# gkm2708/gym-lmaze

Measured on AMD Instinct MI355X. Metric: env steps/sec (whole node), 1M parallel 11x11 mazes at 1/2/4/8 MI355X, higher is better.
Workload: dtype int32

## Files before the change

gym-lmaze_amd/csrc/lmaze_foveal.hip:

```cpp
#include <cstdio>
#include <cstring>
#include <type_traits>

#include "lmaze_foveal_defs.h"

namespace lmaze {

#ifdef LMAZE_FOVEAL_WAVES
#define LMAZE_FOVEAL_ATTR __attribute__((amdgpu_waves_per_eu(LMAZE_FOVEAL_WAVES)))
#else
#define LMAZE_FOVEAL_ATTR
#endif
template <int VARIANT, int MODE, int EPB, int GT, bool AR>
__global__ __launch_bounds__(LMAZE_BLOCK) LMAZE_FOVEAL_ATTR void foveal_kernel(const FovealArgs a) {
    constexpr bool ROLL = false, REC = false;
    const FovealRoll ro{};
#define LMAZE_FOVEAL_BODY_SITE
#include "lmaze_foveal_body.h"
#undef LMAZE_FOVEAL_BODY_SITE
}

template <int VARIANT, int EPB, int GT, bool AR>
__global__ __launch_bounds__(LMAZE_BLOCK) __attribute__((amdgpu_waves_per_eu(4))) void foveal_rollout_kernel(const FovealArgs a, const FovealRoll ro) {
    constexpr bool ROLL = true, REC = false;
    constexpr int MODE = FM_STEP;
#define LMAZE_FOVEAL_BODY_SITE
#include "lmaze_foveal_body.h"
#undef LMAZE_FOVEAL_BODY_SITE
}

template <int VARIANT, int EPB, int GT, bool AR>
__global__ __launch_bounds__(LMAZE_BLOCK)
__attribute__((amdgpu_waves_per_eu(VARIANT == LMAZE_VARIANT_V1 || VARIANT == LMAZE_VARIANT_V2 ? 6 : 4)))
void foveal_rollout_kernel(const FovealArgs a, const FovealRollObs ro) {
    constexpr bool ROLL = true, REC = true;
    constexpr int MODE = FM_STEP;
#define LMAZE_FOVEAL_BODY_SITE
#include "lmaze_foveal_body.h"
#undef LMAZE_FOVEAL_BODY_SITE
}

__global__ __launch_bounds__(LMAZE_BLOCK) void safe_goal_kernel(const FovealArgs a, int32_t* out_goal) {
    const int64_t e = (int64_t)blockIdx.x * LMAZE_BLOCK + threadIdx.x;
    if (e >= a.n) return;
    const int G = a.p.grid;
    const uint8_t* lay = a.layouts + (size_t)clampi(a.b.layout_id[e], 0, a.p.n_layouts - 1) * G * G;
    const int bx = a.b.ball_xy[2 * e], by = a.b.ball_xy[2 * e + 1];
    const uint4 d = env_draw(a.seed, a.epoch, a.env_base + e);
    unsigned ok = 0;
    for (int c = 0; c < W25; ++c) {
        const int x = bx - 2 + c / FOV, y = by - 2 + c % FOV;
        const bool in = x >= 0 && y >= 0 && x < G && y < G;
        if (in && lay[x * G + y] != 'W') ok |= 1u << c;
    }
    int pick = 12;
    const int cnt = __popc(ok);
    if (cnt > 0) {
        int k = (int)__umulhi(d.x, (uint32_t)cnt);
        for (int c = 0; c < W25; ++c)
            if (ok & (1u << c)) {
                if (k == 0) { pick = c; break; }
                --k;
            }
    }
    out_goal[e] = pick;
}

struct ExpandPlanesArgs {
    const float* planes;
    float* out;
    int64_t n;
    int32_t channels, g, expansion;
};

__global__ __launch_bounds__(LMAZE_BLOCK) void expand_planes_kernel(const ExpandPlanesArgs a) {
    extern __shared__ int4 lds4[];
    const int g = a.g, E = a.expansion, C = a.channels;
    const int PC = g * g, S = g * E, PLANE = S * S, L = C * PLANE;
    float* src = reinterpret_cast<float*>(lds4);
    uint16_t* rowmap = reinterpret_cast<uint16_t*>(src + C * PC);
    uint16_t* colmap = rowmap + S;
    const int tid = threadIdx.x;
    for (int64_t i = blockIdx.x; i < a.n; i += gridDim.x) {
        __syncthreads();
        for (int k = tid; k < C * PC; k += LMAZE_BLOCK) src[k] = a.planes[(size_t)i * C * PC + k];
        for (int k = tid; k < S; k += LMAZE_BLOCK) {
            rowmap[k] = (uint16_t)((k / E) * g);
            colmap[k] = (uint16_t)(k / E);
        }
        __syncthreads();
        const size_t B = (size_t)i * L;
        const size_t a0 = (B + 3) & ~(size_t)3, a1 = (B + L) & ~(size_t)3;
        auto value = [&](int local) -> float {
            const int c = local / PLANE;
            const int rem = local - c * PLANE;
            const int row = rem / S, col = rem - row * S;
            return src[c * PC + rowmap[row] + colmap[col]];
        };
        if (tid < (int)(a0 - B)) a.out[B + tid] = value(tid);
        if (tid < (int)(B + L - a1)) a.out[a1 + tid] = value((int)(a1 - B) + tid);
        const int nq = (int)((a1 - a0) >> 2);
        float4* out4 = reinterpret_cast<float4*>(a.out + a0);
        const int head = (int)(a0 - B);
        for (int q = tid; q < nq; q += LMAZE_BLOCK) {
            const int local = head + (q << 2);
            int c = local / PLANE;
            int rem = local - c * PLANE;
            int row = rem / S, col = rem - row * S;
            float v[4];
#pragma unroll
            for (int j = 0; j < 4; ++j) {
                v[j] = src[c * PC + rowmap[row] + colmap[col]];
                if (++col == S) {
                    col = 0;
                    if (++row == S) { row = 0; ++c; }
                }
            }
            out4[q] = make_float4(v[0], v[1], v[2], v[3]);
        }
    }
}

template <int GT, int ET, bool NT>
__global__ __launch_bounds__(LMAZE_BLOCK) void expand_planes_stream_kernel(const ExpandPlanesArgs a, int chunk_floats) {
    constexpr int PC = GT * GT, S = GT * ET, PLANE = S * S;
    extern __shared__ int4 lds4[];
    float* src = reinterpret_cast<float*>(lds4);
    const int tid = threadIdx.x;
    const int64_t total = a.n * (int64_t)a.channels * PLANE;
    const int64_t f0 = (int64_t)blockIdx.x * chunk_floats;
    const int len = (int)min((int64_t)chunk_floats, total - f0);
    const int64_t p0 = f0 / PLANE;
    const int off0 = (int)(f0 - p0 * PLANE);
    const int np = (off0 + len + PLANE - 1) / PLANE;
    for (int k = tid; k < np * PC; k += LMAZE_BLOCK) src[k] = a.planes[(size_t)p0 * PC + k];
    __syncthreads();
    float* dst = a.out + f0;
    static_assert(ET >= 4, "four consecutive output columns span at most two cells");
    for (int q = tid; (q << 2) < len; q += LMAZE_BLOCK) {
        const int local = off0 + (q << 2);
        const int p = local / PLANE;
        const int rem = local - p * PLANE;
        const int row = rem / S, col = rem - row * S;
        const float* r0 = src + p * PC + (row / ET) * GT;
        const int k0 = col / ET;
        const float v0 = r0[k0], v1 = r0[k0 + 1];
        int row1 = row + 1, p1 = p;
        if (row1 == S) { row1 = 0; ++p1; }
        const float vw = src[p1 * PC + (row1 / ET) * GT];
        const int edge = (k0 + 1) * ET;
        float v[4];
#pragma unroll
        for (int j = 0; j < 4; ++j) {
            const int cj = col + j;
            v[j] = cj >= S ? vw : (cj >= edge ? v1 : v0);
        }
        const int count = len - (q << 2);
        if (count >= 4) {
            if (NT) {
                typedef float f4 __attribute__((ext_vector_type(4)));
                f4 t = {v[0], v[1], v[2], v[3]};
                stream_store16(reinterpret_cast<f4*>(dst) + q, t);
            } else {
                reinterpret_cast<float4*>(dst)[q] = make_float4(v[0], v[1], v[2], v[3]);
// ... 517 lines not shown
```

gym-lmaze_amd/csrc/lmaze_foveal_body.h:

```cpp
#ifndef LMAZE_FOVEAL_BODY_SITE
#error "lmaze_foveal_body.h is the body of the foveal kernels: it is included only inside them, in lmaze_foveal.hip and lmaze_foveal_policy.hip"
#endif
#ifdef LMAZE_FOVEAL_POLICY_SITE
#define LMAZE_POL 1
#else
#define LMAZE_POL 0
#endif
    constexpr bool V1 = VARIANT == LMAZE_VARIANT_V1, V5 = VARIANT == LMAZE_VARIANT_V5;
    constexpr bool V4 = VARIANT == LMAZE_VARIANT_V4 || V5;
    constexpr int C = V1 ? 4 : (V4 ? 7 : 5);
    constexpr int PLACE_U = V5 ? 1 : 4;
    constexpr int PERENV = C * W25;
    const int G = GT ? GT : a.p.grid, CELLS = G * G, L = V1 ? 1 : a.p.n_layouts;

    extern __shared__ int4 lds4[];
    uint32_t* obits = reinterpret_cast<uint32_t*>(lds4);
    uint32_t* lbits = obits + EPB * 8;
    int16_t* cen = reinterpret_cast<int16_t*>(lbits + EPB * 4);
    int32_t* flags = reinterpret_cast<int32_t*>(cen + EPB * 4);
    int16_t* rcen = reinterpret_cast<int16_t*>(flags + EPB);
    float* vwin = reinterpret_cast<float*>(rcen + EPB * 2);
    int32_t* clk = reinterpret_cast<int32_t*>(vwin + (V4 ? EPB * 2 * W25 : 0));
    int32_t* dlist = clk + (V4 ? EPB : 0);
    uint64_t* rowfree = reinterpret_cast<uint64_t*>(dlist + (V4 ? EPB : 0));
    uint64_t* rowgoal = rowfree + L * G;
    uint64_t* rowball = rowgoal + L * G;
    uint64_t* rowwall = rowball + L * G;
    uint64_t* rowx = rowwall + G;
    uint8_t* lays = reinterpret_cast<uint8_t*>(rowx + G);
#if LMAZE_POL
    uint8_t* ptab = lays + ((L * CELLS + 15) & ~15);
    const FovealPol pol = ro.pol;
    const bool pstage = pol.in_lds != 0;
#endif
    static_assert(PERENV <= 8 * 32 - 32 && 4 * W25 <= 4 * 32 - 4, "bit strings fit the 32 B / 16 B per env reserved for them");
    __shared__ int any_skip, ndense;

    const int tid = threadIdx.x;
    const int64_t nchunks = (a.n + EPB - 1) / EPB;
    int64_t chunk = blockIdx.x;
    int64_t blockbase = chunk * EPB;
    int nb = (int)min((int64_t)EPB, a.n - blockbase);
    if (tid == 0) { any_skip = 0; ndense = 0; }
    for (int i = tid; i < EPB * 12; i += LMAZE_BLOCK) obits[i] = 0u;
    if (V4) for (int i = tid; i < EPB * 2 * W25; i += LMAZE_BLOCK) vwin[i] = 0.0f;
    const uint64_t epoch = launch_epoch(a.epoch, a.epoch_in);
    if (MODE == FM_STEP && AR) pass_epoch_on(a.epoch_in, a.epoch_out);
    int warmed = 0;
    if (MODE == FM_STEP && !ROLL && a.nt) {
        warmed = warm_lines(a.action, a.n * 4, 256);
        if (!V5 || LMAZE_WARM_V4(a)) {
            warmed += warm_lines(a.b.ball_xy, a.n * 8, 256) + warm_lines(a.b.step_count, a.n * 4, 256);
            if (V1) warmed += warm_lines(a.b.fgoal_xy, a.n * 8, 256) + warm_lines(a.b.foveal_step_count, a.n * 4, 256);
            else warmed += warm_lines(a.b.goal_xy, a.n * 8, 256) + warm_lines(a.b.layout_id, a.n * 4, 256);
            if (V4) warmed += warm_lines(a.b.visit_clock, a.n * 4, 256);
            if (V5) warmed += warm_lines(a.b.fgoal_xy, a.n * 8, 256) + warm_lines(a.b.foveal_step_count, a.n * 4, 256) +
                              warm_lines(a.b.fovea_xy, a.n * 16, 256) + warm_lines(a.b.ball1_xy, a.n * 8, 256) +
                              warm_lines(a.b.last_xy, a.n * 8, 256) + warm_lines(a.b.foveal_goal, a.n * 4, 256) +
                              warm_lines(a.goal2, a.n * 4, 256);
        }
    }
    if (LMAZE_XP(a, 1)) {
    } else if (GT != 0) {
        constexpr int GG = GT ? GT : 1, RPW = 64 / GG, UNR = 8;
        const int wave = tid >> 6, lane = tid & 63, rows = L * G;
        const int rsub = lane / GG, y = lane - rsub * GG;
        const bool dwords = ((reinterpret_cast<uintptr_t>(a.layouts) | (uintptr_t)(L * CELLS)) & 3) == 0;
        uint32_t cw[2] = {0u, 0u};
        if (dwords) {
#pragma unroll
            for (int j = 0; j < 2; ++j)
                if (tid + j * LMAZE_BLOCK < (L * CELLS) >> 2) cw[j] = reinterpret_cast<const uint32_t*>(a.layouts)[tid + j * LMAZE_BLOCK];
        }
#if LMAZE_POL
        const bool pdwords = pstage && ((reinterpret_cast<uintptr_t>(pol.table) | (uintptr_t)(L * CELLS)) & 3) == 0;
        uint32_t pw[2] = {0u, 0u};
        if (pdwords) {
#pragma unroll
            for (int j = 0; j < 2; ++j)
                if (tid + j * LMAZE_BLOCK < (L * CELLS) >> 2) pw[j] = reinterpret_cast<const uint32_t*>(pol.table)[tid + j * LMAZE_BLOCK];
        }
#endif
        for (int r00 = 0; r00 < rows; r00 += UNR * 4 * RPW) {
            uint8_t cc[UNR];
#pragma unroll
            for (int u = 0; u < UNR; ++u) {
                const int row = r00 + (u * 4 + wave) * RPW + rsub;
                cc[u] = (rsub < RPW && row < rows) ? a.layouts[(size_t)row * G + y] : (uint8_t)0;
            }
#pragma unroll
            for (int u = 0; u < UNR; ++u) {
                const int row = r00 + (u * 4 + wave) * RPW + rsub;
                const bool in = rsub < RPW && row < rows;
                const uint8_t c = cc[u];
                const unsigned long long bf = __ballot(in && (c == 'B' || c == 'S' || c == 'X'));
                const unsigned long long bw = __ballot(in && c == 'W');
                const unsigned long long bx = __ballot(in && c == 'X');
                const unsigned long long bs = __ballot(in && c == 'S');
                if (in && y == 0) {
                    const int sh = rsub * GG;
                    const uint64_t keep = GG == 64 ? ~0ull : ((1ull << GG) - 1ull);
                    const uint64_t fr = (bf >> sh) & keep, wl = (bw >> sh) & keep, xx = (bx >> sh) & keep, ss = (bs >> sh) & keep;
                    rowfree[row] = fr;
                    if (V1) { rowwall[row] = wl; rowx[row] = xx; }
                    if (!V1 && (MODE == FM_RESET || (MODE == FM_STEP && AR))) {
                        const int x = row % G;
                        const uint64_t interior = (x >= 1 && x <= G - 2) ? (((1ull << (G - 2)) - 1ull) << 1) : 0ull;
                        rowgoal[row] = fr & ~ss & interior;
                        rowball[row] = fr & ~xx & interior;
                    }
                }
            }
        }
        if (dwords) {
#pragma unroll
            for (int j = 0; j < 2; ++j)
                if (tid + j * LMAZE_BLOCK < (L * CELLS) >> 2) reinterpret_cast<uint32_t*>(lays)[tid + j * LMAZE_BLOCK] = cw[j];
            for (int i = tid + 2 * LMAZE_BLOCK; i < (L * CELLS) >> 2; i += LMAZE_BLOCK)
                reinterpret_cast<uint32_t*>(lays)[i] = reinterpret_cast<const uint32_t*>(a.layouts)[i];
        } else {
            for (int i = tid; i < L * CELLS; i += LMAZE_BLOCK) lays[i] = a.layouts[i];
        }
#if LMAZE_POL
        if (pdwords) {
#pragma unroll
            for (int j = 0; j < 2; ++j)
                if (tid + j * LMAZE_BLOCK < (L * CELLS) >> 2) reinterpret_cast<uint32_t*>(ptab)[tid + j * LMAZE_BLOCK] = pw[j];
            for (int i = tid + 2 * LMAZE_BLOCK; i < (L * CELLS) >> 2; i += LMAZE_BLOCK)
                reinterpret_cast<uint32_t*>(ptab)[i] = reinterpret_cast<const uint32_t*>(pol.table)[i];
        } else if (pstage) {
            for (int i = tid; i < L * CELLS; i += LMAZE_BLOCK) ptab[i] = pol.table[i];
        }
#endif
    } else {
    for (int i = tid; i < L * CELLS; i += LMAZE_BLOCK) lays[i] = a.layouts[i];
#if LMAZE_POL
    if (pstage) for (int i = tid; i < L * CELLS; i += LMAZE_BLOCK) ptab[i] = pol.table[i];
#endif
    __syncthreads();
    for (int i = tid; i < L * G; i += LMAZE_BLOCK) {
        uint64_t fr = 0, wl = 0, xx = 0;
        for (int y = 0; y < G; ++y) {
            const uint8_t c = lays[i * G + y];
            fr |= (uint64_t)(c == 'B' || c == 'S' || c == 'X') << y;
            wl |= (uint64_t)(c == 'W') << y;
            xx |= (uint64_t)(c == 'X') << y;
        }
        rowfree[i] = fr;
        if (V1) { rowwall[i] = wl; rowx[i] = xx; }
        if (!V1 && (MODE == FM_RESET || (MODE == FM_STEP && AR))) {
            uint64_t ss = 0;
            for (int y = 0; y < G; ++y) ss |= (uint64_t)(lays[i * G + y] == 'S') << y;
            const int x = i % G;
            const uint64_t interior = (x >= 1 && x <= G - 2) ? (((1ull << (G - 2)) - 1ull) << 1) : 0ull;
            rowgoal[i] = fr & ~ss & interior;
            rowball[i] = fr & ~xx & interior;
        }
    }
    }
    __syncthreads();

    int t = 0;
#define ROLL_ROW(e) (ROLL ? (int64_t)t * a.n + (e) : (e))
#define ROLL_EP (ROLL ? epoch + (uint64_t)t : epoch)
  for (;;) {
    for (int le = tid; le < (LMAZE_XP(a, 8) ? 0 : nb); le += LMAZE_BLOCK) {
        const int64_t e = blockbase + le;
        EnvRec r;
        r.skip = 0; r.flat = -1; r.action = -1; r.lid = 0; r.gx = r.gy = -9;
        r.b0x = r.b0y = r.b1x = r.b1y = r.f1x = r.f1y = 0; r.upd = 0; r.pad = 0;
        bool fresh = false, nostep = false;
        bool last_is_cur = true;
        int rx = 0, ry = 0;
        float row_r = -0.0f, row_fr = -0.0f;
        int row_d = 0, row_fd = 0;
        int bx = a.b.ball_xy[2 * e], by = a.b.ball_xy[2 * e + 1];
#if LMAZE_POL
        const int act_in = 0;
#else
        const int act_in = (MODE == FM_STEP) ? a.action[ROLL_ROW(e)] : 0;
#endif
        const int sc_ld = (MODE == FM_STEP) ? a.b.step_count[e] : 0;
        const int done_in = (MODE == FM_STEP && AR) ? a.b.done[e] : 0;
        const int goal2_in = (MODE == FM_STEP && AR && V5) ? a.goal2[ROLL_ROW(e)] : 0;
        const int vword = (V4 && !(V5 && MODE == FM_PLANNER)) ? a.b.visit_clock[e] : 0;
        const int vclock = vword & 0xff;
#if LMAZE_POL
        uint4 pr = make_uint4(0u, 0u, 0u, 0u);
        if (pol.epsilon != 0u) pr = policy_draw(a.seed, ROLL_EP, a.env_base + e);
#endif
        r.px = (int16_t)bx; r.py = (int16_t)by;
        if (MODE != FM_STEP && a.mask && !a.mask[e]) r.skip = 1;
        if (V1) {
            int fgx = a.b.fgoal_xy[2 * e], fgy = a.b.fgoal_xy[2 * e + 1];
            r.action = 1;
            if (MODE == FM_STEP) {
                int sc_in = sc_ld;
                if (AR && done_in) {
                    for (int c = 0; c < CELLS; ++c)
                        if (lays[c] == 'S') { bx = c / G; by = c % G; break; }
                    sc_in = 0;
                }
#if LMAZE_POL
                const int act = foveal_pol_action(pol, pstage, ptab, 0, bx, by, G, 1, 4, pr, ROLL_ROW(e));
#else
                const int act = act_in;
#endif
                const int sc = sc_in + 1;
                const int fsc = a.b.foveal_step_count[e] + 1;
                float fr = -0.0f, rw = -0.0f;
                bool local_done = false;
                int ox, oy;
                decode_action(act, ox, oy);
                const int tx = clampi(bx + ox, 0, G - 1), ty = clampi(by + oy, 0, G - 1);
                const uint8_t c = lays[tx * G + ty];
                if (c == 'W') {
                    rw = a.p.reward_wall; fr = a.p.reward_wall;
                } else if (c == 'B') {
                    bx = tx; by = ty;
                    rw = a.p.reward_move; fr = a.p.reward_move;
                    if (bx < fgx - 1 || bx > fgx + 2 || by < fgy - 1 || by > fgy + 2) {
                        local_done = true; fr = a.p.reward_wall;
                    } else if (by == fgy && bx == fgx) {
                        local_done = true; fr = a.p.reward_goal;
                    }
                } else if (c == 'X') {
                    bx = tx; by = ty;
                    rw = a.p.reward_goal;
                    if (by == fgy && bx == fgx) { local_done = true; fr = a.p.reward_goal; }
                    else fr = a.p.reward_move;
                }
                const bool done = (rw == a.p.reward_goal) || (sc == a.p.step_limit);
                const bool fdone = local_done || fr == a.p.reward_goal || fsc == a.p.foveal_step_limit || done;
                a.b.ball_xy[2 * e] = bx; a.b.ball_xy[2 * e + 1] = by;
                a.b.step_count[e] = sc; a.b.foveal_step_count[e] = fsc;
                a.b.reward[e] = rw; a.b.foveal_reward[e] = fr;
                a.b.done[e] = done ? 1 : 0; a.b.foveal_done[e] = fdone ? 1 : 0;
                row_r = rw; row_fr = fr; row_d = done; row_fd = fdone;
            } else if (MODE == FM_RESET && !r.skip) {
                if (a.place) {
                    for (int c = 0; c < CELLS; ++c)
                        if (lays[c] == 'S') { bx = c / G; by = c % G; break; }
                    a.b.ball_xy[2 * e] = bx; a.b.ball_xy[2 * e + 1] = by;
                }
                a.b.reward[e] = -0.0f; a.b.foveal_reward[e] = -0.0f;
                a.b.step_count[e] = 0;
                a.b.done[e] = 0; a.b.foveal_done[e] = 0;
                r.action = 0;
            } else if (MODE == FM_SETGOAL && !r.skip) {
                fgx = bx + a.action[2 * e] - 2;
                fgy = by + a.action[2 * e + 1] - 2;
                a.b.fgoal_xy[2 * e] = fgx; a.b.fgoal_xy[2 * e + 1] = fgy;
                a.b.foveal_step_count[e] = 0;
            }
            int flat = fgx * G + fgy;
            if (flat < 0) flat += CELLS;
            r.flat = (flat >= 0 && flat < CELLS) ? flat : -1;
        } else if (V5) {
            int lid = clampi(a.b.layout_id[e], 0, L - 1);
            int gx = a.b.goal_xy[2 * e], gy = a.b.goal_xy[2 * e + 1];
            int fg = a.b.foveal_goal[e];
            int f0x = a.b.fovea_xy[4 * e], f0y = a.b.fovea_xy[4 * e + 1];
            int f1x = a.b.fovea_xy[4 * e + 2], f1y = a.b.fovea_xy[4 * e + 3];
            int b1x = a.b.ball1_xy[2 * e], b1y = a.b.ball1_xy[2 * e + 1];
            int lx = a.b.last_xy[2 * e], ly = a.b.last_xy[2 * e + 1];
            if (MODE == FM_STEP) {
                const int act = act_in;
                int fgx = a.b.fgoal_xy[2 * e], fgy = a.b.fgoal_xy[2 * e + 1];
                int fsc = a.b.foveal_step_count[e];
                int sc_in = sc_ld;
                bool ld = a.b.foveal_done[e] != 0, gd = a.b.done[e] != 0;
                if (AR) {
                    const bool plan = ld || gd;
                    bool planned = false;
                    if (gd) {
                        const uint4 d = env_draw(a.seed, ROLL_EP, a.env_base + e);
                        lid = (int)__umulhi(d.z, (uint32_t)L);
                        int goal_cell, ball_cell;
                        place_goal_ball<PLACE_U>(rowgoal + lid * G, rowball + lid * G, G, d, goal_cell, ball_cell);
                        if (goal_cell >= 0) { gx = goal_cell / G; gy = goal_cell % G; }
                        if (ball_cell >= 0) { bx = ball_cell / G; by = ball_cell % G; }
                        a.b.layout_id[e] = lid;
                        a.b.goal_xy[2 * e] = gx; a.b.goal_xy[2 * e + 1] = gy;
                        fsc = 0; sc_in = 0; gd = false; ld = false;
                        fg = 12;
                        f0x = f1x = b1x = lx = fgx = bx; f0y = f1y = b1y = ly = fgy = by;
                        fresh = true;
                    }
                    if (plan) {
                        const int g = goal2_in;
                        if (g >= 0 && g < W25) {
                            fg = g;
                            sc_in = 0;
                            ld = false;
                            fgx = bx + g / FOV - 2; fgy = by + g % FOV - 2;
                            if (fsc > 0) { f1x = f0x; f1y = f0y; }
                            fsc += 1;
                            planned = true;
                        }
                    }
                    if (fresh || planned) {
                        a.b.foveal_goal[e] = fg;
                        a.b.fgoal_xy[2 * e] = fgx; a.b.fgoal_xy[2 * e + 1] = fgy;
                        a.b.fovea_xy[4 * e + 2] = f1x; a.b.fovea_xy[4 * e + 3] = f1y;
                        a.b.foveal_step_count[e] = fsc;
                    }
                }
                const uint8_t* lay = lays + lid * CELLS;
                b1x = bx; b1y = by;
                float lr = -0.0f, gr;
                const int sc = sc_in + 1;
                const int dx = (act == 0) - (act == 1), dy = (act == 2) - (act == 3);
                const int nx = bx + dx, ny = by + dy;
                const bool nin = nx >= 0 && ny >= 0 && nx < G && ny < G;
                const uint8_t c = nin ? lay[nx * G + ny] : (uint8_t)'W';
                if (c == 'W') {
                    lr = a.p.reward_wall;
// ... 131 lines not shown
                        if (fx >= G - 2) bx = G - 3;
                        if (fx <= 1) bx = 2;
                        if (fy >= G - 2) by = G - 3;
                        if (fy <= 1) by = 2;
                    }
                    const bool fin = fx >= 0 && fy >= 0 && fx < G && fy < G;
                    const uint8_t c = fin ? lay[fx * G + fy] : (uint8_t)'W';
                    if (fx == gx && fy == gy) rw = a.p.reward_goal;
                    else if (c == 'W') rw = a.p.reward_wall;
                    else if (c == 'B' || c == 'S') rw = a.p.reward_move;
                    a.b.ball_xy[2 * e] = bx; a.b.ball_xy[2 * e + 1] = by;
                    a.b.step_count[e] = sc;
                    a.b.reward[e] = rw;
                    a.b.done[e] = (rw == a.p.reward_goal || sc > a.p.step_limit) ? 1 : 0;
                    r.action = (int16_t)act;
                    row_r = rw; row_d = rw == a.p.reward_goal || sc > a.p.step_limit;
                }
            }
            r.lid = (int16_t)clampi(lid, 0, L - 1);
            r.gx = (int16_t)gx; r.gy = (int16_t)gy;
        }
        r.cx = (int16_t)bx; r.cy = (int16_t)by;
        uint32_t m[8];
        if (V1) {
            m[0] = 1u << 12;
            m[1] = window_bits(rowwall, G, r.cx, r.cy);
            m[2] = r.action ? (r.flat >= 0 ? onehot_bits(r.flat / G, r.flat % G, r.cx, r.cy) : 0u)
                            : window_bits(rowx, G, r.cx, r.cy);
            m[3] = window_bits(rowfree, G, r.cx, r.cy);
        } else {
            constexpr int PER = VARIANT == LMAZE_VARIANT_V2 ? 2 : 3;
            const uint64_t* rows = rowfree + r.lid * G;
            m[0] = window_bits(rows, G, r.cx, r.cy);
            m[1] = onehot_bits(r.gx, r.gy, r.cx, r.cy);
            m[PER] = (r.action >= 0 && r.action < W25) ? (1u << r.action) : 0u;
            m[PER + 1] = window_bits(rows, G, r.px, r.py);
            m[PER + 2] = onehot_bits(r.gx, r.gy, r.px, r.py);
            if (V5) {
                uint32_t lm[4];
                lm[0] = m[0];
                const int i0 = wrap5(r.b0x - r.f1x + 2), j0 = wrap5(r.b0y - r.f1y + 2);
                const int i1 = wrap5(r.b1x - r.f1x + 2), j1 = wrap5(r.b1y - r.f1y + 2);
                lm[1] = (i0 >= 0 && j0 >= 0) ? (1u << (FOV * i0 + j0)) : 0u;
                lm[2] = (i1 >= 0 && j1 >= 0) ? (1u << (FOV * i1 + j1)) : 0u;
                lm[3] = m[PER];
                if (MODE != FM_RESET && !r.skip)
                    for (int ch = 0; ch < 4; ++ch) put_bits(lbits, le * (4 * W25) + ch * W25, lm[ch]);
            }
        }
        if (!r.skip) {
#pragma unroll
            for (int ch = 0; ch < C; ++ch)
                if (!(V4 && (ch == 2 || ch == 6))) put_bits(obits, le * PERENV + ch * W25, m[ch]);
        }
        cen[le * 4 + 0] = r.cx; cen[le * 4 + 1] = r.cy; cen[le * 4 + 2] = r.px; cen[le * 4 + 3] = r.py;
        int fl = (r.skip ? 1 : 0) | (r.upd ? 2 : 0) | (fresh ? 4 : 0) | (nostep ? 8 : 0);
        if (V4 && !(V5 && MODE == FM_PLANNER) && !r.skip) {
            const bool zero = MODE == FM_RESET || (MODE == FM_STEP && AR && fresh);
            const bool renorm = !zero && vclock >= VISIT_RENORM;
            const bool pre = !V5 && MODE == FM_STEP && AR && fresh;
            const bool add = !(V5 && MODE == FM_RESET) && !nostep && !(V5 && MODE == FM_STEP && !r.upd);
            const bool cw0 = V5 && (MODE == FM_RESET || last_is_cur);
            const bool cw1 = V5 && !cw0 && (fresh || add);
            const bool hit = V5 && !zero && (vword >> 8) == (visit_tag(r.px, r.py) >> 8);
            fl |= (zero ? 16 : 0) | (renorm ? 32 : 0) | (pre ? 64 : 0) | (add ? 128 : 0) | (cw0 ? 256 : 0) | (cw1 ? 512 : 0) | (hit ? 1024 : 0);
            int c1 = (zero ? 0 : (renorm ? VISIT_BIAS : vclock)) + (pre ? 1 : 0) + (add ? 1 : 0);
            if (V5) c1 |= cw0 ? visit_tag(r.cx, r.cy) : (cw1 ? visit_tag(r.px, r.py) : (vword & ~0xff));
            if (c1 != vword) a.b.visit_clock[e] = c1;
            if (zero || renorm) dlist[atomicAdd(&ndense, 1)] = le;
        }
        if (V4) clk[le] = vclock;
        flags[le] = fl;
        rcen[le * 2] = (int16_t)rx; rcen[le * 2 + 1] = (int16_t)ry;
        if (r.skip) any_skip = 1;
        if (ROLL) {
            const int64_t o = (int64_t)t * a.n + e;
            if (ro.reward_t) ro.reward_t[o] = row_r;
            if (ro.done_t) ro.done_t[o] = (uint8_t)row_d;
            if (V1 || V5) {
                if (ro.freward_t) ro.freward_t[o] = row_fr;
                if (ro.fdone_t) ro.fdone_t[o] = (uint8_t)row_fd;
            }
        }
    }
    __syncthreads();
    const bool some_skipped = any_skip != 0;

    if (V4 && !(V5 && MODE == FM_PLANNER) && !LMAZE_XP(a, 32)) {
        const int TB = visit_tiles(G), TILES = TB * TB;
        uint32_t* vis = reinterpret_cast<uint32_t*>(a.b.visit) + (size_t)blockbase * TILES * (VT * VT);
        uint32_t* rec = reinterpret_cast<uint32_t*>(a.b.visit) + (size_t)a.n * TILES * (VT * VT) + (size_t)blockbase * VPC;
        auto tile_row_whole = [&](uint32_t (&s)[4], int x, int y0, int le, int fl) {
            const int E0 = clk[le];
            const bool zero = fl & 16, renorm = fl & 32, pre = fl & 64, add = fl & 128;
            const int cx = cen[le * 4], cy = cen[le * 4 + 1], px = cen[le * 4 + 2], py = cen[le * 4 + 3];
            const int E1 = zero ? 0 : (renorm ? VISIT_BIAS : E0);
            const int dx = x - cx + 2, ex = x - px + 2;
#pragma unroll 1
            for (int k = 0; k < 4; ++k) {
                const int y = y0 + k;
                const bool cell_ok = x < G && y < G;
                uint32_t b = s[k];
                if (zero) b = 0u;
                else if (renorm) b = visit_true(b, E0);
                int E = E1;
                if (pre) {
                    const int qx = x - rcen[le * 2] + 2, qy = y - rcen[le * 2 + 1] + 2;
                    if (cell_ok && (unsigned)qx <= 4u && (unsigned)qy <= 4u) b = visit_add(b, E);
                    ++E;
                }
                const int dy = y - cy + 2, ey = y - py + 2;
                const bool in = cell_ok && (unsigned)dx <= 4u && (unsigned)dy <= 4u;
                if (add) {
                    if (in) b = visit_add(b, E);
                    ++E;
                }
                s[k] = b;
                if (in) vwin[le * 2 * W25 + dx * FOV + dy] = __uint_as_float(visit_true(b, E));
                if (cell_ok && (unsigned)ex <= 4u && (unsigned)ey <= 4u)
                    vwin[le * 2 * W25 + W25 + ex * FOV + ey] = __uint_as_float(visit_true(b, E));
            }
        };
        {
            const int nd = ndense, per = TILES * VT;
            for (int j = tid; j < nd * per; j += LMAZE_BLOCK) {
                const int d = j / per, r = j - d * per;
                const int le = dlist[d], fl = flags[le];
                const int tile = r >> 2, row = r & 3;
                const int tx = tile / TB, ty = tile - tx * TB;
                uint32_t* p = vis + (le * TILES + tile) * (VT * VT) + row * VT;
                uint32_t sv[4] = {0u, 0u, 0u, 0u};
                if (!(fl & 16)) {
                    const uint4 t4 = *reinterpret_cast<const uint4*>(p);
                    sv[0] = t4.x; sv[1] = t4.y; sv[2] = t4.z; sv[3] = t4.w;
                }
                tile_row_whole(sv, tx * VT + row, ty * VT, le, fl & 0xff);
                *reinterpret_cast<uint4*>(p) = make_uint4(sv[0], sv[1], sv[2], sv[3]);
            }
        }
        {
#if LMAZE_POL
            constexpr int IPE = 2 * FOV, SUB = EPB < ((REC && !AR) ? 32 : LMAZE_WIN_SUB) ? EPB : ((REC && !AR) ? 32 : LMAZE_WIN_SUB);
            constexpr int NIT = (SUB * IPE + LMAZE_BLOCK - 1) / LMAZE_BLOCK;
#else
            constexpr int IPE = 2 * FOV, SUB = EPB < LMAZE_WIN_SUB ? EPB : LMAZE_WIN_SUB, NIT = (SUB * IPE + LMAZE_BLOCK - 1) / LMAZE_BLOCK;
#endif
          for (int sb = 0; sb < nb; sb += SUB) {
            const int items = LMAZE_XP(a, 256) ? 0 : min(SUB, nb - sb) * IPE;
            uint4 va[NIT], vb[NIT];
            int meta[NIT];
#pragma unroll
            for (int u = 0; u < NIT; ++u) {
                const int i = tid + u * LMAZE_BLOCK;
                meta[u] = -1;
                va[u] = make_uint4(0u, 0u, 0u, 0u);
                vb[u] = make_uint4(0u, 0u, 0u, 0u);
                if (i >= items) continue;
                const int le = sb + i / IPE, r = i % IPE;
                const int w = r >= FOV ? 1 : 0, row = r - w * FOV;
                const int fl = flags[le];
                if (fl & (1 | 16 | 32)) continue;
                const int cx = cen[le * 4], cy = cen[le * 4 + 1];
                const int wx = cen[le * 4 + 2 * w], wy = cen[le * 4 + 2 * w + 1];
                const int x = wx - 2 + row, y0 = wy - 2;
                if ((unsigned)x >= (unsigned)G) continue;
                const bool touched = (fl & 128) && (unsigned)(x - cx + 2) <= 4u && (unsigned)(wy - cy + 4) <= 8u;
                if (V5 && w == 1 && (fl & 1024) && !touched) {
                    const int o = le * VPC + row * FOV;
                    struct __attribute__((packed, aligned(4))) Q4 { uint32_t v[4]; };
                    const Q4 q = *reinterpret_cast<const Q4*>(rec + o);
                    va[u] = make_uint4(q.v[0], q.v[1], q.v[2], q.v[3]);
                    vb[u].x = rec[o + 4];
                    meta[u] = o | (1 << 28);
                } else {
                    const int ty0 = y0 >> 2;
                    const int o = (le * TILES + (x >> 2) * TB + ty0) * (VT * VT) + (x & 3) * VT;
                    const bool a_out = ty0 < 0, b_out = ty0 + 1 >= TB;
                    if (!a_out) va[u] = *reinterpret_cast<const uint4*>(vis + o);
                    if (!b_out) vb[u] = *reinterpret_cast<const uint4*>(vis + o + VT * VT);
                    meta[u] = (o & 0x0fffffff) | (a_out ? 1 << 29 : 0) | (b_out ? 1 << 30 : 0);
                }
            }
            __syncthreads();
#pragma unroll
            for (int u = 0; u < NIT; ++u) {
                if (meta[u] < 0) continue;
                const int i = tid + u * LMAZE_BLOCK;
                const int le = sb + i / IPE, r = i % IPE;
                const int w = r >= FOV ? 1 : 0, row = r - w * FOV;
                const int fl = flags[le], E0 = clk[le];
                const bool add = fl & 128, from_rec = (meta[u] >> 28) & 1;
                const int cx = cen[le * 4], cy = cen[le * 4 + 1];
                const int x = cen[le * 4 + 2 * w] - 2 + row, y0 = cen[le * 4 + 2 * w + 1] - 2;
                const int sh = from_rec ? 0 : (y0 & 3);
                uint32_t c[8] = {va[u].x, va[u].y, va[u].z, va[u].w, vb[u].x, vb[u].y, vb[u].z, vb[u].w};
                if (sh & 1) {
#pragma unroll
                    for (int k = 0; k < 7; ++k) c[k] = c[k + 1];
                }
                if (sh & 2) {
#pragma unroll
                    for (int k = 0; k < 6; ++k) c[k] = c[k + 2];
                }
                const bool rowc = (unsigned)(x - cx + 2) <= 4u;
                bool changed = false;
                float* out = vwin + le * 2 * W25 + w * W25 + row * FOV;
                const bool rec_out = V5 && (fl & (w == 0 ? 256 : 512));
                auto one_cell = [&](uint32_t& cj, int j, bool slow) -> bool {
                    const int y = y0 + j;
                    if ((unsigned)y >= (unsigned)G) return false;
                    const bool in_cur = !from_rec && rowc && (unsigned)(y - cy + 2) <= 4u;
                    const int E = in_cur ? E0 : (from_rec ? VISIT_BIAS : E0) + (add ? 1 : 0);
                    const int n = E - VISIT_BIAS, f = (int)(cj >> 23);
                    const bool fast = cj == 0u || (f >= 1 && f - n >= 1);
                    uint32_t t = slow ? visit_true(cj, E) : (cj == 0u ? 0u : (uint32_t)((int)cj - n * (1 << 23)));
                    if (in_cur && add) {
                        const float nv = (__uint_as_float(t) + 1.0f) * 0.5f;
                        t = __float_as_uint(nv);
                        if (fast || slow) cj = lmaze_visit_store(nv, E0 + 1);
                        changed = true;
                    }
                    out[j] = __uint_as_float(t);
                    if (rec_out) rec[le * VPC + row * FOV + j] = t;
                    return !fast;
                };
                uint32_t redo = 0u;
#pragma unroll
                for (int j = 0; j < FOV; ++j) redo |= one_cell(c[j], j, false) ? 1u << j : 0u;
#pragma unroll 1
                for (; redo; redo &= redo - 1u) {
                    const int j = __ffs((int)redo) - 1;
                    uint32_t cj = j == 0 ? c[0] : (j == 1 ? c[1] : (j == 2 ? c[2] : (j == 3 ? c[3] : c[4])));
                    one_cell(cj, j, true);
                    c[0] = j == 0 ? cj : c[0]; c[1] = j == 1 ? cj : c[1]; c[2] = j == 2 ? cj : c[2];
                    c[3] = j == 3 ? cj : c[3]; c[4] = j == 4 ? cj : c[4];
                }
                if (w == 0 && changed) {
                    uint32_t d[8] = {va[u].x, va[u].y, va[u].z, va[u].w, vb[u].x, vb[u].y, vb[u].z, vb[u].w};
#pragma unroll
                    for (int k = 0; k < 8; ++k) {
#pragma unroll
                        for (int j = 0; j < FOV; ++j)
                            if (k - j >= 0 && k - j <= 3 && sh == k - j) d[k] = c[j];
                    }
                    const int o = meta[u] & 0x0fffffff;
                    if (!((meta[u] >> 29) & 1)) *reinterpret_cast<uint4*>(vis + o) = make_uint4(d[0], d[1], d[2], d[3]);
                    if (!((meta[u] >> 30) & 1)) *reinterpret_cast<uint4*>(vis + o + VT * VT) = make_uint4(d[4], d[5], d[6], d[7]);
                }
            }
            if (V5) {
                for (int i = tid; i < items; i += LMAZE_BLOCK) {
                    const int le = sb + i / IPE, r = i % IPE;
                    const int w = r >= FOV ? 1 : 0, row = r - w * FOV;
                    const int fl = flags[le];
                    if ((fl & (1 | 16 | 32)) || !(fl & (w == 0 ? 256 : 512))) continue;
                    const int x = cen[le * 4 + 2 * w] - 2 + row, y0 = cen[le * 4 + 2 * w + 1] - 2;
                    for (int j = 0; j < FOV; ++j)
                        if ((unsigned)x >= (unsigned)G || (unsigned)(y0 + j) >= (unsigned)G) rec[le * VPC + row * FOV + j] = 0u;
                }
            }
          }
        }
        __syncthreads();
        if (V5) {
            const int nd = ndense;
            for (int j = tid; j < nd * W25; j += LMAZE_BLOCK) {
                const int le = dlist[j / W25], k = j % W25, fl = flags[le];
                if (!(fl & (256 | 512))) continue;
                const int wsel = (fl & 256) ? 0 : 1;
                rec[le * VPC + k] = __float_as_uint(vwin[le * 2 * W25 + wsel * W25 + k]);
            }
        }
    }

    auto element = [&](int le, int rem) -> float {
        if (V4 && rem >= 2 * W25 && rem < 3 * W25) return vwin[le * 2 * W25 + rem - 2 * W25];
        if (V4 && rem >= 6 * W25) return vwin[le * 2 * W25 + rem - 5 * W25];
        const int f = le * PERENV + rem;
        return ((obits[f >> 5] >> (f & 31)) & 1u) ? 1.0f : 0.0f;
    };
    float* obs = a.b.obs + (size_t)blockbase * PERENV;
    const int R = (V5 && MODE == FM_PLANNER) ? 0 : nb * PERENV;
    const int nq = some_skipped ? 0 : (R >> 2);
    if (LMAZE_XP(a, 16) && !V4 && EPB == 128) {
        const int w = blockIdx.x & 7;
        float* gbase = a.b.obs + (size_t)(blockIdx.x >> 3) * 1024 * PERENV;
        const int npieces = 1024 * PERENV / 1024;
        for (int k = 0; k * 8 + w < npieces; ++k) {
            float v[4];
            nibble_floats(obits, (k * 256 + tid) % (EPB * PERENV / 4), v);
            typedef float v4f __attribute__((ext_vector_type(4)));
            v4f t = {v[0], v[1], v[2], v[3]};
            v4f* dst = reinterpret_cast<v4f*>(gbase) + (size_t)(k * 8 + w) * 256 + tid;
            if (a.nt) stream_store16(dst, t); else *dst = t;
        }
    }
    const int nq_run = (LMAZE_XP(a, 4) || (LMAZE_XP(a, 16) && !V4 && EPB == 128)) ? 0 : nq;
    for (int q = tid; q < nq_run; q += LMAZE_BLOCK) {
        const int f = q << 2;
        int le = f / PERENV;
        int rem = f - le * PERENV;
        float v[4];
        if (!V4) {
            nibble_floats(obits, q, v);
        } else {
            nibble_floats(obits, q, v);
            if (rem + 3 >= 2 * W25 && !(rem >= 3 * W25 && rem + 3 < 6 * W25)) {
#pragma unroll
                for (int k = 0; k < 4; ++k) {
                    int r = rem + k, l2 = le;
                    if (r >= PERENV) { r -= PERENV; ++l2; }
                    if (r >= 2 * W25 && r < 3 * W25) v[k] = vwin[l2 * 2 * W25 + r - 2 * W25];
                    else if (r >= 6 * W25) v[k] = vwin[l2 * 2 * W25 + r - 5 * W25];
                }
            }
        }
        if (a.nt) {
            typedef float v4f __attribute__((ext_vector_type(4)));
            v4f t = {v[0], v[1], v[2], v[3]};
            stream_store16(reinterpret_cast<v4f*>(obs) + q, t);
        } else {
            reinterpret_cast<float4*>(obs)[q] = make_float4(v[0], v[1], v[2], v[3]);
        }
        if constexpr (REC) {
            if (float* slot = roll_slot(ro, a.n, blockbase, t, PERENV)) roll_store4(ro, reinterpret_cast<float4*>(slot) + q, v);
        }
    }
    for (int f = (nq << 2) + tid; f < R; f += LMAZE_BLOCK) {
        const int le = f / PERENV;
        if constexpr (REC) {
            if (float* slot = roll_slot(ro, a.n, blockbase, t, PERENV)) {
                if (flags[le] & 1) { slot[f] = obs[f]; continue; }
                const float x = element(le, f - le * PERENV);
                obs[f] = x;
                slot[f] = x;
                continue;
            }
        }
        if (flags[le] & 1) continue;
        obs[f] = element(le, f - le * PERENV);
    }

    if (V5 && MODE != FM_RESET && !LMAZE_XP(a, 4)) {
        constexpr int PERLOC = 4 * W25;
        float* loc = a.b.obs_local + (size_t)blockbase * PERLOC;
        const int RL = nb * PERLOC;
        for (int q = tid; q < (RL >> 2); q += LMAZE_BLOCK) {
            const int f = q << 2;
            const int le = f / PERLOC;
            if constexpr (REC) {
                float* lslot = roll_lslot(ro, a.n, blockbase, t);
                if (lslot && (flags[le] & 1)) {
                    reinterpret_cast<float4*>(lslot)[q] = reinterpret_cast<const float4*>(loc)[q];
                    continue;
                }
            }
            if (flags[le] & 1) continue;
            float v[4];
            nibble_floats(lbits, q, v);
            if constexpr (REC) {
                if (float* lslot = roll_lslot(ro, a.n, blockbase, t)) roll_store4(ro, reinterpret_cast<float4*>(lslot) + q, v);
            }
            if (a.nt) {
                typedef float v4f __attribute__((ext_vector_type(4)));
                v4f t = {v[0], v[1], v[2], v[3]};
                stream_store16(reinterpret_cast<v4f*>(loc) + q, t);
            } else {
                reinterpret_cast<float4*>(loc)[q] = make_float4(v[0], v[1], v[2], v[3]);
            }
        }
    }
    if (ROLL && ++t < ro.T) {
        asm volatile("s_waitcnt vmcnt(0)" ::: "memory");
    } else {
        t = 0;
        chunk += gridDim.x;
        if (chunk >= nchunks) break;
        blockbase = chunk * EPB;
        nb = (int)min((int64_t)EPB, a.n - blockbase);
    }
    __syncthreads();
    for (int i = tid; i < EPB * 12; i += LMAZE_BLOCK) obits[i] = 0u;
    if (V4) for (int i = tid; i < EPB * 2 * W25; i += LMAZE_BLOCK) vwin[i] = 0.0f;
    if (tid == 0) { any_skip = 0; ndense = 0; }
    __syncthreads();
  }
    if (warmed == 0x7fedcba9 && a.n < 0) a.b.done[0] = 1;
#undef ROLL_ROW
#undef ROLL_EP
#undef LMAZE_POL
```

gym-lmaze_amd/csrc/lmaze_foveal_defs.h:

```cpp
#ifndef LMAZE_FOVEAL_DEFS_H_
#define LMAZE_FOVEAL_DEFS_H_

#include "lmaze_common.h"
#include "lmaze_visit.h"
#include "lmaze_foveal_select.h"

#ifdef LMAZE_EXPERIMENT
#define LMAZE_WARM_V4(args) ((((args).p.launch_hint >> 16) & 1024) != 0)
#define LMAZE_XP(args, mask) ((((args).p.launch_hint >> 16) & (mask)) != 0)
#else
#define LMAZE_WARM_V4(args) false
#define LMAZE_XP(args, mask) false
#endif

namespace lmaze {

constexpr int FOV = LMAZE_FOVEA;
constexpr int W25 = FOV * FOV;

enum FovealMode { FM_STEP = 0, FM_RESET = 1, FM_SETGOAL = 2, FM_PLANNER = 3 };

struct FovealArgs {
    LmazeFovealParams p;
    LmazeFovealBuffers b;
// ... 14 lines not shown

struct FovealRoll {
    int32_t T;
    float* reward_t;
    uint8_t* done_t;
    float* freward_t;
    uint8_t* fdone_t;
};

struct FovealRollObs : FovealRoll {
    float* obs_t;
    float* obs_local_t;
    int32_t every;
};

__device__ __forceinline__ float* roll_slot(const FovealRoll&, int64_t, int64_t, int, int) { return nullptr; }
__device__ __forceinline__ float* roll_slot(const FovealRollObs& ro, int64_t n, int64_t base, int t, int per) {
    if (ro.obs_t == nullptr || (t + 1) % ro.every != 0) return nullptr;
    return ro.obs_t + ((size_t)((t + 1) / ro.every - 1) * n + base) * per;
}
__device__ __forceinline__ float* roll_lslot(const FovealRoll&, int64_t, int64_t, int) { return nullptr; }
__device__ __forceinline__ float* roll_lslot(const FovealRollObs& ro, int64_t n, int64_t base, int t) {
    if (ro.obs_local_t == nullptr || (t + 1) % ro.every != 0) return nullptr;
    return ro.obs_local_t + ((size_t)((t + 1) / ro.every - 1) * n + base) * (4 * W25);
}
__device__ __forceinline__ void roll_store4(const FovealRoll&, float4*, const float*) {}
__device__ __forceinline__ void roll_store4(const FovealRollObs&, float4* p, const float* v) {
    *p = make_float4(v[0], v[1], v[2], v[3]);
}

struct FovealPol {
    const uint8_t* table;
    uint32_t epsilon;
    int32_t in_lds;
    int32_t* actions_t;
    int32_t* key_t;
};
struct FovealRollPol : FovealRoll { FovealPol pol; };
struct FovealRollObsPol : FovealRollObs { FovealPol pol; };
__device__ __forceinline__ int foveal_pol_action(const FovealPol& pol, bool staged, const uint8_t* lds_table, int lid, int bx, int by,
                                                 int G, int L, int A, const uint4& r, int64_t row) {
    typedef const __attribute__((address_space(3))) uint8_t* lds_bytes;
    typedef const __attribute__((address_space(1))) uint8_t* global_bytes;
    const int key = lmaze_foveal_key(lid, bx, by, G, L);
    const int greedy = staged ? (int)((lds_bytes)lds_table)[key] : (int)((global_bytes)pol.table)[key];
    const int act = lmaze_foveal_choose(greedy, r.x, r.y, pol.epsilon, A);
    if (pol.actions_t) pol.actions_t[row] = act;
    if (pol.key_t) pol.key_t[row] = key;
    return act;
}
constexpr int kFovealPolicyLds = 8192;
hipError_t launch_foveal_rollout_policy(const FovealArgs& a, const FovealRollObsPol& ro, bool rec, hipStream_t s);

struct EnvRec {
    int16_t cx, cy;
    int16_t px, py;
    int16_t gx, gy;
    int16_t lid;
    int16_t action;
    int32_t skip;
    int32_t flat;
    int16_t b0x, b0y;
    int16_t b1x, b1y;
    int16_t f1x, f1y;
    int16_t upd;
    int16_t pad;
};


template <int U>
__device__ __forceinline__ void mask_counts(const uint64_t* goal_rows, const uint64_t* ball_rows, int G, int& cg, int& cb) {
    cg = 0; cb = 0;
#pragma unroll U
    for (int x = 1; x <= G - 2; ++x) { cg += __popcll(goal_rows[x]); cb += __popcll(ball_rows[x]); }
}

template <int U>
__device__ __forceinline__ int mask_kth(const uint64_t* rows, int G, int k, int hole) {
    int xr = -1, kk = 0, acc = 0;
#pragma unroll U
    for (int x = 1; x <= G - 2; ++x) {
        uint64_t m = rows[x];
        const unsigned hy = (unsigned)(hole - x * G);
        if (hy < (unsigned)G) m &= ~(1ull << hy);
        const int c = __popcll(m);
        if (xr < 0 && k < acc + c) { xr = x; kk = k - acc; }
        acc += c;
    }
    if (xr < 0) return -1;
    uint64_t m = rows[xr];
    const unsigned hy = (unsigned)(hole - xr * G);
    if (hy < (unsigned)G) m &= ~(1ull << hy);
    uint32_t h = (uint32_t)m;
    int base = 0;
    const int cl = __popc(h);
    if (kk >= cl) { kk -= cl; h = (uint32_t)(m >> 32); base = 32; }
    for (; kk > 0; --kk) h &= h - 1;
    return xr * G + base + (__ffs((int)h) - 1);
}

template <int U>
__device__ __forceinline__ void place_goal_ball(const uint64_t* goal_rows, const uint64_t* ball_rows, int G, uint4 d,
                                                int& goal_cell, int& ball_cell) {
    goal_cell = -1;
    ball_cell = -1;
    int cg, cb;
    mask_counts<U>(goal_rows, ball_rows, G, cg, cb);
    if (cg > 0) goal_cell = mask_kth<U>(goal_rows, G, (int)__umulhi(d.x, (uint32_t)cg), -1);
    if (goal_cell >= 0 && ((ball_rows[goal_cell / G] >> (goal_cell % G)) & 1ull)) --cb;
    if (cb > 0) ball_cell = mask_kth<U>(ball_rows, G, (int)__umulhi(d.y, (uint32_t)cb), goal_cell);
}

__device__ __forceinline__ int wrap5(int i) {
    if (i >= 0 && i < FOV) return i;
    if (i < 0 && i >= -FOV) return i + FOV;
    return -1;
}

__device__ __forceinline__ uint32_t window_bits(const uint64_t* rows, int G, int cx, int cy) {
    uint32_t m = 0;
    const int y0 = cy - 2;
#pragma unroll
    for (int i = 0; i < FOV; ++i) {
        const int x = cx - 2 + i;
        const uint64_t b = (x >= 0 && x < G) ? rows[x] : 0ull;
        const uint32_t w = (uint32_t)(y0 >= 0 ? (b >> y0) : (b << -y0)) & 31u;
        m |= w << (FOV * i);
    }
    return m;
}

__device__ __forceinline__ uint32_t onehot_bits(int tx, int ty, int cx, int cy) {
    const int i = tx - cx + 2, j = ty - cy + 2;
    return (i >= 0 && i < FOV && j >= 0 && j < FOV) ? (1u << (FOV * i + j)) : 0u;
}

__device__ __forceinline__ void put_bits(uint32_t* bits, int off, uint32_t m) {
    const int w = off >> 5, sh = off & 31;
    atomicOr(&bits[w], m << sh);
    if (sh > 32 - W25) atomicOr(&bits[w + 1], m >> (32 - sh));
}

__device__ __forceinline__ void lds_dma16(const uint32_t* src, uint32_t* lds_wave_base) {
    typedef __attribute__((address_space(1))) void gvoid;
    typedef __attribute__((address_space(3))) void lvoid;
    __builtin_amdgcn_global_load_lds((gvoid*)src, (lvoid*)lds_wave_base, 16, 0, 0);
}

__device__ __forceinline__ void nibble_floats(const uint32_t* bits, int q, float (&v)[4]) {
    const uint32_t nib = bits[q >> 3] >> ((q & 7) << 2);
#pragma unroll
    for (int k = 0; k < 4; ++k) v[k] = __uint_as_float((0u - ((nib >> k) & 1u)) & 0x3f800000u);
}

constexpr int VISIT_BIAS = LMAZE_VISIT_BIAS, VISIT_RENORM = LMAZE_VISIT_RENORM;
constexpr int VT = 4;
constexpr int VPC = 28;
__host__ __device__ __forceinline__ int visit_tag(int x, int y) { return 0x100 | ((x & 0x7f) << 9) | ((y & 0x7f) << 16); }

__host__ __device__ __forceinline__ int visit_tiles(int G) { return (G + VT - 1) / VT; }
__device__ __forceinline__ uint32_t visit_true(uint32_t bits, int E) { return lmaze_visit_true(bits, E); }
__device__ __forceinline__ uint32_t visit_add(uint32_t bits, int E) { return lmaze_visit_add(bits, E); }

#ifndef LMAZE_WIN_SUB
#define LMAZE_WIN_SUB 64
#endif

constexpr size_t kFovealStreamBytes = (size_t)192 << 20;

static inline size_t lds_limit() {
    static size_t limit = 0;
    if (limit == 0) {
        int dev = 0, v = 0;
        if (hipGetDevice(&dev) == hipSuccess && hipDeviceGetAttribute(&v, hipDeviceAttributeMaxSharedMemoryPerBlock, dev) == hipSuccess && v > 0)
            limit = (size_t)v;
        else
            limit = 64 * 1024;
    }
    return limit;
}

template <int VARIANT>
static size_t foveal_lds(const LmazeFovealParams& p, int epb) {
    const int cells = p.grid * p.grid;
    const int L = VARIANT == LMAZE_VARIANT_V1 ? 1 : p.n_layouts;
    size_t lds = (size_t)epb * 64 + (3 * (size_t)L * p.grid + 2 * (size_t)p.grid) * 8 + (size_t)((L * cells + 15) & ~15);
    if (VARIANT == LMAZE_VARIANT_V4 || VARIANT == LMAZE_VARIANT_V5)
        lds += (size_t)epb * (2 * W25 * 4 + 8);
    return lds;
}

static inline size_t lds_for_cap(size_t lds, int per_cu) {
    if (per_cu >= 1 && per_cu <= 8) {
        const size_t cap = 160 * 1024;
        const size_t want = ((cap / per_cu + cap / (per_cu + 1)) / 2) & ~(size_t)255;
        if (want > lds && want <= lds_limit()) return want;
    }
    return lds;
}

static inline int check_foveal(const LmazeFovealParams* p, const uint8_t* layouts, const LmazeFovealBuffers* b, int64_t n) {
    if (!p || !layouts || !b) return LMAZE_E_NULL;
    const bool v56 = p->variant == LMAZE_VARIANT_V5 || p->variant == LMAZE_VARIANT_V6;
    if (p->variant != LMAZE_VARIANT_V1 && p->variant != LMAZE_VARIANT_V2 && p->variant != LMAZE_VARIANT_V4 && !v56)
        return LMAZE_E_VARIANT;
    if (p->grid < FOV || p->grid > LMAZE_MAX_GRID) return LMAZE_E_GRID;
    if (p->n_layouts < 1 || p->n_layouts > LMAZE_MAX_LAYOUTS) return LMAZE_E_LAYOUT;
    if (n < 0 || n > LMAZE_MAX_ENVS) return LMAZE_E_COUNT;
#ifndef LMAZE_EXPERIMENT
    if (p->launch_hint & ~0x3ff) return LMAZE_E_LAYOUT;
#endif
    if (v56) {
        if (!b->fgoal_xy || !b->foveal_step_count || !b->foveal_reward || !b->foveal_done || !b->visit || !b->ball1_xy ||
            !b->fovea_xy || !b->last_xy || !b->foveal_goal || !b->obs_local)
            return LMAZE_E_NULL;
        if ((uintptr_t)b->obs_local & 15) return LMAZE_E_ALIGN;
    }
    if (!b->ball_xy || !b->step_count || !b->reward || !b->done || !b->obs) return LMAZE_E_NULL;
    if (p->variant == LMAZE_VARIANT_V1 && (!b->fgoal_xy || !b->foveal_step_count || !b->foveal_reward || !b->foveal_done))
        return LMAZE_E_NULL;
    if (p->variant != LMAZE_VARIANT_V1 && (!b->goal_xy || !b->layout_id)) return LMAZE_E_NULL;
    if ((p->variant == LMAZE_VARIANT_V4 || v56) && (!b->visit || !b->visit_clock)) return LMAZE_E_NULL;
    if (((uintptr_t)b->obs & 15) || (b->visit && ((uintptr_t)b->visit & 63))) return LMAZE_E_ALIGN;
    return 0;
}

static inline FovealArgs make_foveal_args(const LmazeFovealParams* p, const uint8_t* layouts, const LmazeFovealBuffers* b, int64_t n) {
    FovealArgs a;
    a.p = *p;
    a.b = *b;
    a.layouts = layouts;
    a.action = nullptr;
    a.goal2 = nullptr;
    a.mask = nullptr;
    a.n = n;
    a.place = 0;
    a.seed = 0;
    a.epoch = 0;
    a.env_base = 0;
    a.epoch_in = nullptr;
    a.epoch_out = nullptr;
    a.nt = 0;
    a.auto_reset = 0;
    a.info = nullptr;
    return a;
}

}

#endif
```

Measured before the change: 13.64 billion.

## Overlap local-obs stores with window loads and make the window loads branchless

In the flat V4/V5 step path, the window-gather loop now issues unconditional 16-byte loads, using clamped in-bounds pointers instead of per-item branches. For V5 it moves the obs_local nibble-to-float writeback into the gap between those loads and the barrier, splitting the stores evenly across sub-batches. The later separate writeback pass is skipped. The default waves-per-eu attribute is now 4 for the V5 step autoreset fixed-grid kernel and 1 otherwise, which changes register allocation and occupancy for all other instantiations.

```diff
diff --git a/gym-lmaze_amd/csrc/lmaze_foveal.hip b/gym-lmaze_amd/csrc/lmaze_foveal.hip
--- a/gym-lmaze_amd/csrc/lmaze_foveal.hip
+++ b/gym-lmaze_amd/csrc/lmaze_foveal.hip
@@ -9,7 +9,8 @@
 #ifdef LMAZE_FOVEAL_WAVES
 #define LMAZE_FOVEAL_ATTR __attribute__((amdgpu_waves_per_eu(LMAZE_FOVEAL_WAVES)))
 #else
-#define LMAZE_FOVEAL_ATTR
+#define LMAZE_FOVEAL_ATTR \
+    __attribute__((amdgpu_waves_per_eu(VARIANT == LMAZE_VARIANT_V5 && MODE == FM_STEP && AR && GT != 0 ? 4 : 1)))
 #endif
 template <int VARIANT, int MODE, int EPB, int GT, bool AR>
 __global__ __launch_bounds__(LMAZE_BLOCK) LMAZE_FOVEAL_ATTR void foveal_kernel(const FovealArgs a) {
diff --git a/gym-lmaze_amd/csrc/lmaze_foveal_body.h b/gym-lmaze_amd/csrc/lmaze_foveal_body.h
--- a/gym-lmaze_amd/csrc/lmaze_foveal_body.h
+++ b/gym-lmaze_amd/csrc/lmaze_foveal_body.h
@@ -9,6 +9,7 @@
     constexpr bool V1 = VARIANT == LMAZE_VARIANT_V1, V5 = VARIANT == LMAZE_VARIANT_V5;
     constexpr bool V4 = VARIANT == LMAZE_VARIANT_V4 || V5;
     constexpr int C = V1 ? 4 : (V4 ? 7 : 5);
+    constexpr bool FLAT = V4 && MODE == FM_STEP && !ROLL && !LMAZE_POL, EARLY = FLAT && V5;
     constexpr int PLACE_U = V5 ? 1 : 4;
     constexpr int PERENV = C * W25;
     const int G = GT ? GT : a.p.grid, CELLS = G * G, L = V1 ? 1 : a.p.n_layouts;
@@ -163,6 +164,7 @@
     int t = 0;
 #define ROLL_ROW(e) (ROLL ? (int64_t)t * a.n + (e) : (e))
 #define ROLL_EP (ROLL ? epoch + (uint64_t)t : epoch)
+#define LMAZE_EARLY_ON (EARLY && !some_skipped && !LMAZE_XP(a, 32 | 64))
   for (;;) {
     for (int le = tid; le < (LMAZE_XP(a, 8) ? 0 : nb); le += LMAZE_BLOCK) {
         const int64_t e = blockbase + le;
@@ -600,6 +602,41 @@
 #pragma unroll
             for (int u = 0; u < NIT; ++u) {
                 const int i = tid + u * LMAZE_BLOCK;
+                if constexpr (FLAT) {
+                    struct __attribute__((packed, aligned(4))) Q4 { uint32_t v[4]; };
+                    const uint32_t* pa = vis;
+                    const uint32_t* pb = vis;
+                    int m = -1;
+                    if (i < items) {
+                        const int le = sb + i / IPE, r = i % IPE;
+                        const int w = r >= FOV ? 1 : 0, row = r - w * FOV;
+                        const int fl = flags[le];
+                        const int cx = cen[le * 4], cy = cen[le * 4 + 1];
+                        const int wx = cen[le * 4 + 2 * w], wy = cen[le * 4 + 2 * w + 1];
+                        const int x = wx - 2 + row, y0 = wy - 2;
+                        if (!(fl & (1 | 16 | 32)) && (unsigned)x < (unsigned)G) {
+                            const bool touched = (fl & 128) && (unsigned)(x - cx + 2) <= 4u && (unsigned)(wy - cy + 4) <= 8u;
+                            if (V5 && w == 1 && (fl & 1024) && !touched) {
+                                const int o = le * VPC + row * FOV;
+                                pa = rec + o;
+                                pb = rec + o + 4;
+                                m = o | (1 << 28);
+                            } else {
+                                const int ty0 = y0 >> 2;
+                                const int o = (le * TILES + (x >> 2) * TB + ty0) * (VT * VT) + (x & 3) * VT;
+                                const bool a_out = ty0 < 0, b_out = ty0 + 1 >= TB;
+                                pa = vis + (a_out ? o + VT * VT : o);
+                                pb = vis + (b_out ? o : o + VT * VT);
+                                m = (o & 0x0fffffff) | (a_out ? 1 << 29 : 0) | (b_out ? 1 << 30 : 0);
+                            }
+                        }
+                    }
+                    const Q4 qa = *reinterpret_cast<const Q4*>(pa), qb = *reinterpret_cast<const Q4*>(pb);
+                    va[u] = make_uint4(qa.v[0], qa.v[1], qa.v[2], qa.v[3]);
+                    vb[u] = make_uint4(qb.v[0], qb.v[1], qb.v[2], qb.v[3]);
+                    meta[u] = m;
+                    continue;
+                }
                 meta[u] = -1;
                 va[u] = make_uint4(0u, 0u, 0u, 0u);
                 vb[u] = make_uint4(0u, 0u, 0u, 0u);
@@ -629,6 +666,23 @@
                     meta[u] = (o & 0x0fffffff) | (a_out ? 1 << 29 : 0) | (b_out ? 1 << 30 : 0);
                 }
             }
+            if constexpr (EARLY) {
+                if (LMAZE_EARLY_ON && !LMAZE_XP(a, 4)) {
+                    const int np = (nb + SUB - 1) / SUB, p = sb / SUB;
+                    float* const eloc = a.b.obs_local + (size_t)blockbase * (4 * W25);
+                    const int enl = nb * W25;
+                    constexpr int IT_LOC = (SUB * W25 + LMAZE_BLOCK) / LMAZE_BLOCK;
+                    static_assert(IT_LOC * LMAZE_BLOCK > SUB * W25, "a share plus its rounding");
+LMAZE_EARLY_PRAGMA
+                    for (int k = 0; k < IT_LOC; ++k) {
+                        const int q = enl * p / np + tid + k * LMAZE_BLOCK;
+                        if (q >= enl * (p + 1) / np || (flags[q / W25] & 1)) continue;
+                        float v[4];
+                        nibble_floats(lbits, q, v);
+                        store_piece(eloc, q, v, a.nt != 0);
+                    }
+                }
+            }
             __syncthreads();
 #pragma unroll
             for (int u = 0; u < NIT; ++u) {
@@ -789,7 +843,7 @@
         obs[f] = element(le, f - le * PERENV);
     }
 
-    if (V5 && MODE != FM_RESET && !LMAZE_XP(a, 4)) {
+    if (V5 && MODE != FM_RESET && !LMAZE_XP(a, 4) && !LMAZE_EARLY_ON) {
         constexpr int PERLOC = 4 * W25;
         float* loc = a.b.obs_local + (size_t)blockbase * PERLOC;
         const int RL = nb * PERLOC;
@@ -836,4 +890,5 @@
     if (warmed == 0x7fedcba9 && a.n < 0) a.b.done[0] = 1;
 #undef ROLL_ROW
 #undef ROLL_EP
+#undef LMAZE_EARLY_ON
 #undef LMAZE_POL
diff --git a/gym-lmaze_amd/csrc/lmaze_foveal_defs.h b/gym-lmaze_amd/csrc/lmaze_foveal_defs.h
--- a/gym-lmaze_amd/csrc/lmaze_foveal_defs.h
+++ b/gym-lmaze_amd/csrc/lmaze_foveal_defs.h
@@ -190,6 +190,25 @@
 #pragma unroll
     for (int k = 0; k < 4; ++k) v[k] = __uint_as_float((0u - ((nib >> k) & 1u)) & 0x3f800000u);
 }
+
+__device__ __forceinline__ void store_piece(float* base, int q, const float (&v)[4], bool nt) {
+    if (nt) {
+        typedef float v4f __attribute__((ext_vector_type(4)));
+        v4f t = {v[0], v[1], v[2], v[3]};
+        stream_store16(reinterpret_cast<v4f*>(base) + q, t);
+    } else {
+        reinterpret_cast<float4*>(base)[q] = make_float4(v[0], v[1], v[2], v[3]);
+    }
+}
+
+#ifndef LMAZE_EARLY_UNROLL
+#define LMAZE_EARLY_UNROLL 1
+#endif
+#if LMAZE_EARLY_UNROLL
+#define LMAZE_EARLY_PRAGMA _Pragma("unroll")
+#else
+#define LMAZE_EARLY_PRAGMA _Pragma("unroll 1")
+#endif
 
 constexpr int VISIT_BIAS = LMAZE_VISIT_BIAS, VISIT_RENORM = LMAZE_VISIT_RENORM;
 constexpr int VT = 4;
```

After: 13.48 billion. -1.1%, worse.
